# juanaldayparejo/archnemesis-dist

Hardware: AMD Instinct MI355X
Metric: forward-models/sec (10k nu x 100 layers) (higher is better)
Workload: dtype f64; 1 GPU; synthetic correlated-k nadir thermal-emission forward model: 10000 wavenumbers x 100 layers x 8 gases, G=20, k-table 20Px15T (BASELINE configs[1], SURVEY C2); parallelism=replicas x1 (independent forward models)

## Files before the change

archnemesis_dist_amd/csrc/ansfm_api.hip:

```cpp
#include "ansfm_table_kernels.hip.h"
#include "ansfm_rt_params.h"
#include "ansfm_ctx.hip.h"

using namespace ansfm;

extern "C" {

int ansfm_abi_version(void) { return ANSFM_ABI_VERSION; }

int ansfm_create(int device, ansfm_ctx **out)
{
    if (!out) return ANSFM_ERR_INVALID;
    *out = nullptr;
    int ndev = 0;
    if (hipGetDeviceCount(&ndev) != hipSuccess || ndev <= 0 || device < 0 || device >= ndev)
        return ANSFM_ERR_HIP;
    ansfm_ctx *ctx = new ansfm_ctx();
    ctx->device = device;
    if (hipSetDevice(device) != hipSuccess) { delete ctx; return ANSFM_ERR_HIP; }
    if (hipStreamCreateWithFlags(&ctx->own_stream, hipStreamNonBlocking) != hipSuccess) {
        delete ctx;
        return ANSFM_ERR_HIP;
    }
    ctx->stream = ctx->own_stream;
// ... 26 lines not shown
int ansfm_set_gradient_gases(ansfm_ctx *ctx, unsigned int mask)
{
    CHECK_CTX(ctx);
    ctx->grad_gas_mask = mask;
    return ANSFM_OK;
}

int ansfm_set_f32_semantics(ansfm_ctx *ctx, int grid_f32, int delg_f32)
{
    CHECK_CTX(ctx);
    ctx->grid_f32 = grid_f32 ? 1 : 0;
    ctx->delg_f32 = delg_f32 ? 1 : 0;
    return ANSFM_OK;
}

int ansfm_synchronize(ansfm_ctx *ctx)
{
    CHECK_CTX(ctx);
    HIPCHK(hipSetDevice(ctx->device));
    HIPCHK(hipStreamSynchronize(ctx->stream));
    return ANSFM_OK;
}

int ansfm_upload_ktable_dev(ansfm_ctx *ctx, int W, int G, int NP, int NT, int S, const double *K_dev,
                            const double *PRESS, const double *TEMP, const double *WAVE,
                            const double *DELG)
{
    CHECK_CTX(ctx);
    if (W <= 0 || G <= 0 || G > ANSFM_MAX_NG || NP < 2 || NT < 2 || S <= 0 || !K_dev || !PRESS || !TEMP ||
        !WAVE || !DELG)
        FAIL(ANSFM_ERR_INVALID, "upload_ktable: bad dims (need 1<=G<=32, NP>=2, NT>=2) or null pointer");
    HIPCHK(hipSetDevice(ctx->device));
    const int Wpad = round_up(W, kWave);
    const size_t total = (size_t)NP * NT * S * G * Wpad;
    HIPCHK(ctx->lnK.reserve(total * sizeof(double)));
    HIPCHK(ctx->d_press.reserve(NP * sizeof(double)));
    HIPCHK(ctx->d_temp.reserve(NT * sizeof(double)));
    HIPCHK(ctx->d_wave.reserve((size_t)W * sizeof(double)));
    HIPCHK(ctx->d_delg.reserve(kMaxG * sizeof(double)));
    HIPCHK(ctx->d_flag.reserve(kFlagInts * sizeof(int)));
    HIPCHK(hipMemcpyAsync(ctx->d_press.p, PRESS, NP * sizeof(double), hipMemcpyHostToDevice, ctx->stream));
    HIPCHK(hipMemcpyAsync(ctx->d_temp.p, TEMP, NT * sizeof(double), hipMemcpyHostToDevice, ctx->stream));
    HIPCHK(hipMemcpyAsync(ctx->d_wave.p, WAVE, (size_t)W * sizeof(double), hipMemcpyHostToDevice, ctx->stream));
    HIPCHK(hipMemcpyAsync(ctx->d_delg.p, DELG, G * sizeof(double), hipMemcpyHostToDevice, ctx->stream));
    HIPCHK(hipMemsetAsync(ctx->d_flag.p, 0, kFlagInts * sizeof(int), ctx->stream));
    {
        const int Q = NP * NT * S;
        hipLaunchKernelGGL(k_table_check, dim3(nblk((size_t)W * Q, 256)), dim3(256), 0, ctx->stream, K_dev, W, G, Q,
                           ctx->d_flag.as<int>());
        hipLaunchKernelGGL(k_table_relayout, dim3((unsigned)(Wpad / kWave), nblk((size_t)Q, 64), (unsigned)G), dim3(256), 0,
                           ctx->stream, K_dev, ctx->lnK.as<double>(), W, Wpad, G, Q);
    }
    HIPCHK(hipGetLastError());
    int flag = 0;
    HIPCHK(hipMemcpyAsync(&flag, ctx->d_flag.p, sizeof(int), hipMemcpyDeviceToHost, ctx->stream));
    HIPCHK(hipStreamSynchronize(ctx->stream));
    ctx->W = W; ctx->Wpad = Wpad; ctx->G = G; ctx->NP = NP; ctx->NT = NT; ctx->S = S;
    ctx->monotone = (flag & 1) ? 0 : 1;
    ctx->has_boxed = (flag & 2) ? 1 : 0;
    ctx->h_delg.assign(DELG, DELG + G);
    ctx->h_wave.assign(WAVE, WAVE + W); ctx->h_press.assign(PRESS, PRESS + NP); ctx->h_temp.assign(TEMP, TEMP + NT);
    ctx->have_table = true;
    ctx->is_lbl = 0; ctx->temp2d = 0;
    ctx->lblrt = 0; ctx->st_n = 0;
    clear_continuum_sources(ctx);
    return ANSFM_OK;
}

int ansfm_upload_ktable(ansfm_ctx *ctx, int W, int G, int NP, int NT, int S, const double *K,
                        const double *PRESS, const double *TEMP, const double *WAVE, const double *DELG)
{
    CHECK_CTX(ctx);
    if (W <= 0 || G <= 0 || NP <= 0 || NT <= 0 || S <= 0 || !K) FAIL(ANSFM_ERR_INVALID, "upload_ktable: bad dims");
    HIPCHK(hipSetDevice(ctx->device));
    const size_t n = (size_t)W * G * NP * NT * S;
    HIPCHK(ctx->tmp_in.reserve(n * sizeof(double)));
    HIPCHK(hipMemcpyAsync(ctx->tmp_in.p, K, n * sizeof(double), hipMemcpyHostToDevice, ctx->stream));
    int rc = ansfm_upload_ktable_dev(ctx, W, G, NP, NT, S, ctx->tmp_in.as<double>(), PRESS, TEMP, WAVE, DELG);
    ctx->tmp_in.release();
    return rc;
}

namespace {
struct KtaHeader {
    int irec0 = 0, nwave = 0, npress = 0, ntemp = 0, ng = 0, gasID = 0, isoID = 0;
    double vmin = 0, delv = 0, fwhm = 0;
    std::vector<float> g_ord, del_g, press, temp;
    std::vector<double> wave;
    bool temp2d = false;
// ... 119 lines not shown
            FAIL(ANSFM_ERR_INVALID, "upload_ktable_files: " + err);
        if (hs[s].nwave != hs[0].nwave) FAIL(ANSFM_ERR_INVALID, "error :: Number of wavenumbers in all .kta files must be the same");
        if (hs[s].npress != hs[0].npress) FAIL(ANSFM_ERR_INVALID, "error :: Number of pressure levels in all .kta files must be the same");
        if (hs[s].ntemp != hs[0].ntemp) FAIL(ANSFM_ERR_INVALID, "error :: Number of temperature levels in all .kta files must be the same");
        if (hs[s].ng != hs[0].ng) FAIL(ANSFM_ERR_INVALID, "error :: Number of g-ordinates in all .kta files must be the same");
        if (hs[s].temp2d != hs[0].temp2d) FAIL(ANSFM_ERR_INVALID, "error :: Number of temperature levels in all .kta files must be the same");
    }
    const KtaHeader &hl = hs[S - 1];
    const int G = hl.ng, NP = hl.npress, NT = hl.ntemp;
    if (G > ANSFM_MAX_NG || NP < 2 || NT < 2) FAIL(ANSFM_ERR_INVALID, "upload_ktable_files: need 1<=G<=32, NP>=2, NT>=2");
    if (lta && NP > 256) FAIL(ANSFM_ERR_UNSUPPORTED, "upload_lbltable_files: NP <= 256");
    const std::vector<double> &wv = hl.wave;
    long iwl = (long)(std::upper_bound(wv.begin(), wv.end(), wavemin) - wv.begin()) - 1;
    if (iwl < 0) iwl = 0;
    long iwh = (long)(std::lower_bound(wv.begin(), wv.end(), wavemax) - wv.begin());
    if (iwh >= (long)wv.size()) iwh = (long)wv.size() - 1;
    if (iwh < iwl) FAIL(ANSFM_ERR_INVALID, "upload_ktable_files: empty wavenumber range");
    const double wlo = wv[iwl], whi = wv[iwh];
    const int W = (int)(iwh - iwl + 1);
    std::vector<double> WAVE(wv.begin() + iwl, wv.begin() + iwh + 1), PRESS(hl.press.begin(), hl.press.end()),
        TEMP(hl.temp.begin(), hl.temp.end()), DELG(hl.del_g.begin(), hl.del_g.end());
    const int Wpad = round_up(W, kWave);
    const size_t total = (size_t)NP * NT * S * G * Wpad;
    HIPCHK(ctx->lnK.reserve(total * sizeof(double)));
    HIPCHK(ctx->d_press.reserve(NP * sizeof(double)));
    HIPCHK(ctx->d_temp.reserve(TEMP.size() * sizeof(double)));
    HIPCHK(ctx->d_wave.reserve((size_t)W * sizeof(double)));
    HIPCHK(ctx->d_delg.reserve(kMaxG * sizeof(double)));
    HIPCHK(ctx->d_flag.reserve(kFlagInts * sizeof(int)));
    HIPCHK(hipMemcpyAsync(ctx->d_press.p, PRESS.data(), NP * sizeof(double), hipMemcpyHostToDevice, ctx->stream));
    HIPCHK(hipMemcpyAsync(ctx->d_temp.p, TEMP.data(), TEMP.size() * sizeof(double), hipMemcpyHostToDevice, ctx->stream));
    HIPCHK(hipMemcpyAsync(ctx->d_wave.p, WAVE.data(), (size_t)W * sizeof(double), hipMemcpyHostToDevice, ctx->stream));
    HIPCHK(hipMemcpyAsync(ctx->d_delg.p, DELG.data(), G * sizeof(double), hipMemcpyHostToDevice, ctx->stream));
    HIPCHK(hipMemsetAsync(ctx->d_flag.p, 0, kFlagInts * sizeof(int), ctx->stream));
    const size_t per_wave = (size_t)NP * NT * G;
    std::vector<float> block(per_wave * W);
    HIPCHK(ctx->tmp_in.reserve(block.size() * sizeof(float)));
    for (int s = 0; s < S; ++s) {
        const std::vector<double> &ws = hs[s].wave;
        const long a = (long)(std::lower_bound(ws.begin(), ws.end(), wlo) - ws.begin());
        const long b = (long)(std::upper_bound(ws.begin(), ws.end(), whi) - ws.begin());
        if (b - a != W) FAIL(ANSFM_ERR_INVALID, "upload_ktable_files: the tables do not share one wavenumber grid");
        std::string fn(paths[s]);
        const char *ext = lta ? ".lta" : ".kta";
        if (fn.size() < 4 || fn.compare(fn.size() - 4, 4, ext) != 0) fn += ext;
        FILE *f = fopen(fn.c_str(), "rb");
// ... 2 lines not shown
        const bool ok = fseeko(f, (off_t)off, SEEK_SET) == 0 && fread(block.data(), 4, block.size(), f) == block.size();
        fclose(f);
        if (!ok) FAIL(ANSFM_ERR_INVALID, "upload_ktable_files: truncated k data in " + fn);
        HIPCHK(hipMemcpyAsync(ctx->tmp_in.p, block.data(), block.size() * sizeof(float), hipMemcpyHostToDevice, ctx->stream));
        hipLaunchKernelGGL(k_kta_relayout, dim3(nblk(per_wave * Wpad, 256)), dim3(256), 0, ctx->stream, ctx->tmp_in.as<float>(),
                           ctx->lnK.as<double>(), W, Wpad, G, NP, NT, S, s, ctx->d_flag.as<int>());
        HIPCHK(hipGetLastError());
        HIPCHK(hipStreamSynchronize(ctx->stream));
    }
    int flag = 0;
    HIPCHK(hipMemcpyAsync(&flag, ctx->d_flag.p, sizeof(int), hipMemcpyDeviceToHost, ctx->stream));
    HIPCHK(hipStreamSynchronize(ctx->stream));
    ctx->tmp_in.release();
    ctx->W = W; ctx->Wpad = Wpad; ctx->G = G; ctx->NP = NP; ctx->NT = NT; ctx->S = S;
    ctx->monotone = (flag & 1) ? 0 : 1;
    ctx->has_boxed = (flag & 2) ? 1 : 0;
    ctx->h_delg = DELG; ctx->h_wave = WAVE; ctx->h_press = PRESS; ctx->h_temp = TEMP;
    ctx->have_table = true;
    ctx->is_lbl = lta ? 1 : 0; ctx->temp2d = (lta && hl.temp2d) ? 1 : 0;
    ctx->lblrt = 0; ctx->st_n = 0;
    clear_continuum_sources(ctx);
    if (lta) ctx->monotone = 1;
    ctx->grid_f32 = 1; ctx->delg_f32 = lta ? 0 : 1;
    return ANSFM_OK;
}

int ansfm_upload_ktable_files(ansfm_ctx *ctx, int S, const char *const *paths, double wavemin, double wavemax)
{
    return upload_table_files(ctx, S, paths, wavemin, wavemax, false);
}

int ansfm_upload_lbltable_files(ansfm_ctx *ctx, int S, const char *const *paths, double wavemin, double wavemax)
{
    return upload_table_files(ctx, S, paths, wavemin, wavemax, true);
}

int ansfm_ktable_grids(const ansfm_ctx *ctx, double *WAVE, double *PRESS, double *TEMP, double *DELG)
{
    if (!ctx) return ANSFM_ERR_INVALID;
    if (!ctx->have_table) return ANSFM_ERR_NOTABLE;
    if (WAVE) memcpy(WAVE, ctx->h_wave.data(), ctx->h_wave.size() * sizeof(double));
    if (PRESS) memcpy(PRESS, ctx->h_press.data(), ctx->h_press.size() * sizeof(double));
    if (TEMP) memcpy(TEMP, ctx->h_temp.data(), ctx->h_temp.size() * sizeof(double));
    if (DELG) memcpy(DELG, ctx->h_delg.data(), ctx->h_delg.size() * sizeof(double));
    return ANSFM_OK;
}

// ... 6 lines not shown
    return ANSFM_OK;
}

int ansfm_ktable_has_boxed(const ansfm_ctx *ctx, int *has_boxed)
{
    if (!ctx || !has_boxed) return ANSFM_ERR_INVALID;
    if (!ctx->have_table) return ANSFM_ERR_NOTABLE;
    *has_boxed = ctx->has_boxed;
    return ANSFM_OK;
}

int ansfm_last_merge_launch(const ansfm_ctx *ctx, int *waves_per_block, int *trims)
{
    if (!ctx || !waves_per_block || !trims) return ANSFM_ERR_INVALID;
    *waves_per_block = ctx->merge_block_waves;
    *trims = ctx->merge_trims;
    return ANSFM_OK;
}

int ansfm_last_merge_group_width(const ansfm_ctx *ctx, int *width)
{
    if (!ctx || !width) return ANSFM_ERR_INVALID;
    *width = ctx->merge_group_width;
    return ANSFM_OK;
}

int ansfm_last_merge_rowmajor(const ansfm_ctx *cctx, int64_t *merges, int64_t *merges_total)
{
    ansfm_ctx *ctx = const_cast<ansfm_ctx *>(cctx);
    CHECK_CTX(ctx);
    if (!merges || !merges_total) FAIL(ANSFM_ERR_INVALID, "last_merge_rowmajor: null argument");
    *merges = *merges_total = 0;
    if (ctx->d_flag.bytes < kFlagInts * sizeof(int)) return ANSFM_OK;
    HIPCHK(hipSetDevice(ctx->device));
    unsigned long long v[2] = {0, 0};
    HIPCHK(hipMemcpyAsync(v, ctx->d_flag.as<int>() + kFlagTileCounter + 8, sizeof v, hipMemcpyDeviceToHost, ctx->stream));
    HIPCHK(hipStreamSynchronize(ctx->stream));
    *merges = (int64_t)v[0];
    *merges_total = (int64_t)v[1];
    return ANSFM_OK;
}

static void launch_w_to_last(hipStream_t st, unsigned n_batch, const double *src, double *dst, int W, int Wpad, int X1, int X2,
                             int swap12, double padval, size_t src_stride = 0, size_t dst_stride = 0)
{
    const int X = X1 * X2;
// ... 1020 lines not shown
```

archnemesis_dist_amd/csrc/ansfm_ctx.hip.h:

```cpp
#pragma once
#include <hip/hip_runtime.h>
#include <stdio.h>
#include <stdlib.h>
#include <string.h>

#include <algorithm>
#include <cmath>
#include <initializer_list>
#include <memory>
#include <string>
#include <map>
#include <vector>

#pragma GCC visibility push(default)
#include "../../include/ansfm.h"
#pragma GCC visibility pop

namespace ansfm {

struct DevBuf {
    void *p = nullptr;
    size_t bytes = 0;
    DevBuf() = default;
    DevBuf(const DevBuf &) = delete;
// ... 42 lines not shown

struct ansfm_ctx {
    int device = 0;
    hipStream_t own_stream = nullptr;
    hipStream_t stream = nullptr;
    std::string err;
    int num_cus = 256;

    int W = 0, Wpad = 0, G = 0, NP = 0, NT = 0, S = 0;
    int monotone = 0;
    int has_boxed = 1;
    std::vector<double> h_wave, h_press, h_temp;
    DevBuf dcont_gas;
    int dcont_gas_L = 0;
    unsigned grad_gas_mask = 0xFFFFFFFFu;
    std::map<const void *, size_t> merge_lds_allowed;
    int merge_block_waves = 0, merge_trims = 0;
    int merge_group_width = 0;
    int merge_keys = 64;
    bool have_table = false;
    int grid_f32 = 0, delg_f32 = 0;
    int is_lbl = 0, temp2d = 0;
    DevBuf lnK, d_press, d_temp, d_wave, d_delg, d_flag;
    std::vector<double> h_delg;
    DevBuf cia_tab, cia_idx, cia_lay, dust_kext;
    int cia_on = 0, cia_ispace = 0, cia_NWC = 0, cia_NPAIR = 0, cia_NPE = 0, cia_NT = 0, cia_nfrac = 0, cia_NPARA = 0, cia_NVMR = 0,
        cia_ico2 = -1, cia_in2 = -1, cia_ih2 = -1, cia_covers = 0;
    int dust_n = 0;

    DevBuf li, tau, scratch, cont_t, tmp_in, tmp_out, misc;
    DevBuf dspec_ref, map_out, map_b, map_batch;
    DevBuf dd_slot, dd_work, dd_in;
    DevBuf ms_radg16, ms_brdf16;
    DevBuf rt_prefix, rt_same;
    int last_rt_shared = 0;
    int dedup = 1;
    int last_rows = 0, last_dedup = 0;
    int dspec_dims[4] = {0, 0, 0, 0};
    int map_dims[4] = {0, 0, 0, 0};
    DevBuf gscratch, perm, dkbuf, trold_ws, dspec_i, dcont_t, tmp_in2, tmp_out2, lbl_li;
    DevBuf ms_taus, ms_omegas, ms_bnu;
    DevBuf ms_tauray_l, ms_lfrac_l;
    DevBuf ms_cache, ms_orders, ms_same, ms_pcache, ms_lstart;
    long ms_cache_hits = 0, ms_cache_layers = 0;
    long ms_windows = 0, ms_window_w = 0;
    DevBuf hb[24];
// ... 147 lines not shown
```

archnemesis_dist_amd/csrc/ansfm_merge64.hip.h:

```cpp
#pragma once
#include <hip/hip_runtime.h>
#include <stdint.h>
#include "ansfm_merge_common.hip.h"

namespace ansfm {

constexpr unsigned kLdsDG = 0, kLdsGORD = kMaxG * 8, kLdsDGF = (2 * kMaxG + 2) * 8, kLdsA = kLdsDGF + kMaxG * 4;


constexpr int kOptTable = 1, kOptBfi = 2, kOptExit = 8, kOptOrient = 16;
constexpr int kMergeOpt = kOptTable | kOptBfi | kOptExit | kOptOrient;
constexpr int kOptLaneRows = 32;
constexpr int kOptRowMajor = 64;
constexpr int kFlagLaneRows = 1, kFlagRowMajor = 2;
__host__ __device__ constexpr bool merge_opt_valid(int opt) { return opt == 0 || (opt & ~kOptTable) == (kOptBfi | kOptExit | kOptOrient); }
__host__ __device__ constexpr int merge_wave_rows(int G, int opt) { return 2 * G + ((opt & kOptOrient) != 0 ? 2 : 1); }
constexpr unsigned kLdsWT = kLdsA;
constexpr int kMaxBlockWaves = 8;
__host__ __device__ constexpr unsigned weight_table_bytes(int G) { return (unsigned)(G + 1) * 32u * 8u; }
typedef double dbl2 __attribute__((ext_vector_type(2)));
constexpr unsigned kRecRow = 64u * 16u, kRecBin = 2u * kRecRow;

struct MergeElem {
    double ai, bc, bn, w;
    int ci, np;
};

struct MergeOrient {
    unsigned rbase, cbase;
    unsigned rsh, csh;
    unsigned inc;
};
__device__ __forceinline__ MergeOrient merge_orient(unsigned a_addr, unsigned b_addr, bool swapped)
{
    MergeOrient mo;
    mo.rbase = swapped ? b_addr : a_addr; mo.cbase = swapped ? a_addr : b_addr;
    mo.rsh = swapped ? 6u : 0u; mo.csh = swapped ? 0u : 5u; mo.inc = swapped ? 1u : 32u;
// ... 349 lines not shown
```

archnemesis_dist_amd/csrc/ansfm_merge_common.hip.h:

```cpp
#pragma once
#include <hip/hip_runtime.h>
#include <stdint.h>

namespace ansfm {

constexpr int kWave = 64;
constexpr int kMaxG = 32;

__device__ __forceinline__ double encode_lnk(double k)
{
    if (k > 0.0) return log(k);
    unsigned long long b = (unsigned long long)__double_as_longlong(k);
    unsigned long long box = 0x7FF8000000000000ULL | (b >> 13);
    return __longlong_as_double((long long)box);
}
__device__ __forceinline__ bool lnk_is_boxed(double x) { return x != x; }
__device__ __forceinline__ double lnk_unbox(double x)
{
    unsigned long long b = (unsigned long long)__double_as_longlong(x);
    return __longlong_as_double((long long)((b & 0x0007FFFFFFFFFFFFULL) << 13));
}

struct LayerInterp {
    int ipl, iph, itl, ith;
// ... 38 lines not shown
        double dxdt = (-l1 * (1.0 - v) - h1 * v + h2 * v + l2 * (1.0 - v)) * dudt;
        dk = kk * dxdt;
    } else if (b1 & b2 & b3 & b4) {
        double klo1 = lnk_unbox(l1), klo2 = lnk_unbox(l2), khi1 = lnk_unbox(h1), khi2 = lnk_unbox(h2);
        kk = (1.0 - v) * (1.0 - u) * klo1 + v * (1.0 - u) * khi1 + v * u * khi2 + (1.0 - v) * u * klo2;
        dk = (-klo1 * (1.0 - v) - khi1 * v + khi2 * v + klo2 * (1.0 - v)) * dudt;
    }
}


struct OverlapParams {
    const double *lnK;
    const double *kin;
    const LayerInterp *li;
    const double *amount;
    const double *del_g;
    double *tau;
    double *scratch;
    int *err_flag;
    unsigned int *tile_counter;
    int W, Wpad, G, NT, S, L, n_models;
    int delg_f32;
    double g_ord[kMaxG + 2];
};


constexpr int kLoadBatch = 10;

template <bool FROM_K, bool NONNEG = false, bool NOBOX = false>
__device__ __forceinline__ void load_gas(const OverlapParams &p, const LayerInterp &q, int m, int l,
                                         int s, int nu, double *DST, int lane, bool &unsorted)
{
    const int G = p.G;
    const double amt = p.amount[((size_t)m * p.S + s) * p.L + l];
    double prev = NONNEG ? 0.0 : -__builtin_inf();
    if constexpr (FROM_K) {
        const double *src = p.kin + (((size_t)s * p.L + l) * G) * p.Wpad + nu;
        for (int g0 = 0; g0 < G; g0 += kLoadBatch) {
            double r[kLoadBatch];
#pragma unroll
            for (int k = 0; k < kLoadBatch; ++k) {
                const int gi = (g0 + k < G) ? g0 + k : G - 1;
                r[k] = src[(size_t)gi * p.Wpad];
            }
#pragma unroll
            for (int k = 0; k < kLoadBatch; ++k)
                if (g0 + k < G) {
// ... 85 lines not shown
    {0, 0, 100, 2, 0, 0}, {1, 36, 100, 2, 0, 50}, {99, 63, 100, 2, 63, 99}, {50, 17, 100, 2, 33, 8},
    {1, 36, 33, 1, 3, 1}, {32, 63, 33, 1, 63, 32}, {16, 17, 33, 1, 31, 18}, {1, 36, 3, 2, 32, 2}, {2, 63, 3, 2, 63, 2}, {1, 17, 3, 2, 27, 1}};
__host__ __device__ constexpr bool lane_spots_hold()
{
    for (const auto &t : kLaneTileSpots)
        if ((t[2] != 1u && t[2] != (unsigned)kLaneNV) || lane_tile_of(t[0], t[1], t[2] == 1u ? 0u : kLaneNVShift) != t[3]) return false;
    for (const auto &t : kLaneCellSpots) {
        if (t[3] != 1u && t[3] != (unsigned)kLaneNV) return false;
        const LaneCell x = lane_cell(t[0] * 64u + t[1], t[2], t[3] == 1u ? 0u : kLaneNVShift);
        if (x.w != t[4] || x.row != t[5]) return false;
    }
    return true;
}
static_assert(lane_spots_hold(), "lane_tile_of / lane_cell against the model's values");

struct LaneRow {
    int nu;
    unsigned row;
    unsigned arow, krow;
    size_t o1, o2, o3, o4;
    double v, u;
};
template <bool FROM_K>
__device__ __forceinline__ LaneRow lane_row(const OverlapParams &p, int vt, unsigned k, int lane, unsigned nvs)
{
    const unsigned R = (unsigned)p.n_models * (unsigned)p.L;
    const LaneCell cell = lane_cell(k * kWave + (unsigned)lane, R, nvs);
    LaneRow lr;
    lr.row = cell.row;
    lr.nu = vt * kWave + (int)cell.w;
    const unsigned m = lr.row / (unsigned)p.L;
    lr.krow = lr.row - m * (unsigned)p.L;
    lr.arow = m * (unsigned)p.S * (unsigned)p.L + lr.krow;
    lr.o1 = lr.o2 = lr.o3 = lr.o4 = 0;
    lr.v = lr.u = 0.0;
    if constexpr (!FROM_K) {
        const LayerInterp q = p.li[lr.row];
        const size_t strideT = (size_t)p.S * p.G * p.Wpad;
        lr.o1 = ((size_t)q.ipl * p.NT + q.itl) * strideT + lr.nu;
        lr.o2 = ((size_t)q.ipl * p.NT + q.ith) * strideT + lr.nu;
        lr.o3 = ((size_t)q.iph * p.NT + q.itl) * strideT + lr.nu;
        lr.o4 = ((size_t)q.iph * p.NT + q.ith) * strideT + lr.nu;
        lr.v = q.v; lr.u = q.u;
    }
    return lr;
}

template <bool FROM_K, bool NOBOX>
__device__ __forceinline__ void load_gas_rows(const OverlapParams &p, const LaneRow &lr, int s, double *DST, int lane,
                                              bool &unsorted)
{
    const int G = p.G;
    const double amt = p.amount[(size_t)lr.arow + (size_t)s * p.L];
    double prev = -__builtin_inf();
    if constexpr (FROM_K) {
        const double *src = p.kin + (((size_t)s * p.L + lr.krow) * G) * p.Wpad + lr.nu;
        for (int g0 = 0; g0 < G; g0 += kLoadBatch) {
            double r[kLoadBatch];
#pragma unroll
            for (int k = 0; k < kLoadBatch; ++k) {
                const int gi = (g0 + k < G) ? g0 + k : G - 1;
                r[k] = src[(size_t)gi * p.Wpad];
            }
#pragma unroll
            for (int k = 0; k < kLoadBatch; ++k)
                if (g0 + k < G) {
                    const double kk = r[k] * amt;
                    DST[(g0 + k) * kWave + lane] = kk;
                    unsorted |= (kk < prev);
                    prev = kk;
                }
        }
    } else {
        const double *base = p.lnK + (size_t)s * G * p.Wpad;
        const double *c1 = base + lr.o1, *c2 = base + lr.o2, *c3 = base + lr.o3, *c4 = base + lr.o4;
        for (int g0 = 0; g0 < G; g0 += kLoadBatch) {
            double r1[kLoadBatch], r2[kLoadBatch], r3[kLoadBatch], r4[kLoadBatch];
#pragma unroll
            for (int k = 0; k < kLoadBatch; ++k) {
                const int gi = (g0 + k < G) ? g0 + k : G - 1;
                const size_t go = (size_t)gi * p.Wpad;
                r1[k] = c1[go];
                r2[k] = c2[go];
                r3[k] = c3[go];
                r4[k] = c4[go];
            }
#pragma unroll
            for (int k = 0; k < kLoadBatch; ++k)
                if (g0 + k < G) {
                    const double kk = (NOBOX ? interp_k_nobox(r1[k], r2[k], r3[k], r4[k], lr.v, lr.u)
                                             : interp_k(r1[k], r2[k], r3[k], r4[k], lr.v, lr.u)) * amt;
                    DST[(g0 + k) * kWave + lane] = kk;
                    unsorted |= (kk < prev);
                    prev = kk;
                }
        }
    }
}

__device__ __forceinline__ double fast_div(double n, double d)
{
    double r = __builtin_amdgcn_rcp(d);
    r = fma(fma(-d, r, 1.0), r, r);
    r = fma(fma(-d, r, 1.0), r, r);
    double q = n * r;
    return fma(fma(-d, q, n), r, q);
}

// ... 71 lines not shown
```

archnemesis_dist_amd/csrc/ansfm_overlap.hip:

```cpp
#include "ansfm_overlap_kernels.hip.h"
#include "ansfm_merge32_launch.h"
#include "ansfm_ctx.hip.h"

namespace ansfm {

void merge_params(ansfm_ctx *ctx, OverlapParams &p, const double *kin, int W, int Wpad, int G, int S, int L, int n_models,
                  const LayerInterp *li, const double *amount, const double *del_g_dev, const double *del_g_host, double *tau)
{
    p.lnK = ctx->lnK.as<double>();
    p.kin = kin;
    p.li = li;
    p.amount = amount;
    p.del_g = del_g_dev;
    p.tau = tau;
    p.err_flag = ctx->d_flag.as<int>() + 1;
    p.tile_counter = reinterpret_cast<unsigned int *>(ctx->d_flag.as<int>() + kFlagTileCounter);
    p.W = W; p.Wpad = Wpad; p.G = G; p.NT = ctx->NT; p.S = S; p.L = L; p.n_models = n_models;
    p.delg_f32 = ctx->delg_f32;
    double acc = 0.0;
    float accf = 0.0f;
    p.g_ord[0] = 0.0;
    for (int g = 0; g < G; ++g) {
        if (ctx->delg_f32) { accf += (float)del_g_host[g]; p.g_ord[g + 1] = (double)accf; }
        else { acc += del_g_host[g]; p.g_ord[g + 1] = acc; }
// ... 56 lines not shown
    if ((opt & kOptTable) != 0) {
        const size_t shared_bytes = table_bytes + weight_table_bytes(G);
        nwaves = (int)((kCuLdsBytes - shared_bytes) / wave_bytes);
        if (nwaves > max_per_cu) nwaves = max_per_cu;
        if (nwaves > kMaxBlockWaves) nwaves = kMaxBlockWaves;
        lds = shared_bytes + (size_t)nwaves * wave_bytes;
        const int rc = merge_launch_begin(ctx, p, lds, 1, {{&ctx->scratch, (size_t)nwaves * 6 * G * kWave * sizeof(double)}}, &grid);
        if (rc) return rc;
        const long ntiles = (long)n_models * (Wpad / kWave) * L;
        if (grid > (ntiles + nwaves - 1) / nwaves) grid = (ntiles + nwaves - 1) / nwaves;
    } else {
        const int rc = merge_launch_begin(ctx, p, lds_alloc, max_per_cu, {{&ctx->scratch, (size_t)6 * G * kWave * sizeof(double)}}, &grid);
        if (rc) return rc;
    }
    p.scratch = ctx->scratch.as<double>();
    bool lane_rows = opt != 0 && (long)n_models * L < (1L << 24);
    int lane_nv = 1;
    if (const char *ev = getenv("ANSFM_MERGE_LANES")) {
        if (!strcmp(ev, "wavenumbers")) lane_rows = false;
        else if (!strcmp(ev, "pairs")) lane_nv = kLaneNV;
    }
    bool rowmajor = (opt & kOptTable) != 0;
    if (const char *ev = getenv("ANSFM_MERGE_ROWMAJOR")) { if (ev[0] == '0') rowmajor = false; }
    const int flags = (lane_rows ? kFlagLaneRows : 0) | (rowmajor ? kFlagRowMajor : 0);
    ctx->merge_block_waves = nwaves;
    ctx->merge_group_width = lane_rows ? lane_nv : 0;
    ctx->merge_trims = opt == 0 ? 0 : merge_opt_of(ctx->delg_f32 != 0) | (lane_rows ? kOptLaneRows : 0) | (rowmajor ? kOptRowMajor : 0);
    if (keys32) {
        HIPCHK(launch_overlap32(p, from_k, merge_list_len(G), (unsigned)grid, ctx->stream));
        return ANSFM_OK;
    }
#define LAUNCH_OPT(...)                                                                                             \
    do {                                                                                                            \
        auto kern = __VA_ARGS__;                                                                                    \
        size_t &lds_allowed = ctx->merge_lds_allowed[reinterpret_cast<const void *>(kern)];     \
        if (lds > (size_t)64 * 1024 && lds > lds_allowed) {          \
            HIPCHK(hipFuncSetAttribute(reinterpret_cast<const void *>(kern), hipFuncAttributeMaxDynamicSharedMemorySize, (int)lds)); \
            lds_allowed = lds;                                                                                      \
        }                                                                                                           \
        hipLaunchKernelGGL(kern, dim3((unsigned)grid), dim3(kWave * nwaves), lds, ctx->stream, p, flags, lane_nv);           \
    } while (0)
#define LAUNCH_OV2(D, FK, W32)                                                                                      \
    do {                                                                                                            \
        if (opt != 0 && nobox)                                                                                      \
            LAUNCH_OPT(k_ck_overlap<D, false, W32, true, true, true, merge_opt_of(W32)>);                           \
        else if (opt != 0)                                                                                          \
            LAUNCH_OPT(k_ck_overlap<D, FK, W32, true, true, false, merge_opt_of(W32)>);                             \
// ... 32 lines not shown
```

archnemesis_dist_amd/csrc/ansfm_overlap_kernels.hip.h:

```cpp
#pragma once
#include "ansfm_merge64.hip.h"

namespace ansfm {


template <bool FROM_K, bool NOBOX, int OPT>
__device__ __forceinline__ void load_cell(const OverlapParams &p, int lane_rows, const LaneRow &lr, const LayerInterp &q, int m,
                                          int l, int s, int nu, double *DST, int lane, bool &unsorted)
{
    if constexpr (OPT != 0) {
        if (lane_rows != 0) {
            load_gas_rows<FROM_K, NOBOX>(p, lr, s, DST, lane, unsorted);
            return;
        }
    }
    load_gas<FROM_K, false, NOBOX>(p, q, m, l, s, nu, DST, lane, unsorted);
}

template <int NR, bool FROM_K, bool W32, bool SORTED = true, bool NODIV = false, bool NOBOX = false, int OPT = 0>
__global__ __launch_bounds__((OPT & kOptTable) != 0 ? kWave * kMaxBlockWaves : kWave) __attribute__((amdgpu_waves_per_eu(1, 2)))
void k_ck_overlap(OverlapParams p, int flags, int lane_nv)
{
    static_assert(OPT == 0 || (SORTED && NODIV), "the fast path");
    static_assert(merge_opt_valid(OPT), "OPT == 0 || (OPT & ~kOptTable) == (kOptBfi | kOptExit | kOptOrient)");
    constexpr bool kTable = (OPT & kOptTable) != 0, kOrient = (OPT & kOptOrient) != 0;
    static_assert(!kTable || W32, "the weight table holds float32 products only (launch_overlap)");
    const int lane_rows = kTable ? (flags & kFlagLaneRows) : flags;
    const unsigned nvs = lane_nv == 1 ? 0u : kLaneNVShift;
    unsigned n_rowmajor = 0, n_merged = 0;
    extern __shared__ double smem[];
    const int lane = kTable ? (int)(threadIdx.x & 63u) : (int)threadIdx.x;
    const int wv = kTable ? __builtin_amdgcn_readfirstlane((int)(threadIdx.x >> 6)) : 0;
    const int nwv = kTable ? (int)(blockDim.x >> 6) : 1;
    const int G = p.G;
    double *DG = smem;
    double *GORD = DG + kMaxG;
    double *A = reinterpret_cast<double *>(reinterpret_cast<char *>(GORD + kMaxG + 2) + kMaxG * sizeof(float));
    if constexpr (kTable) {
        double *WT = A;
        for (int idx = (int)threadIdx.x; idx < (G + 1) * 32; idx += (int)blockDim.x) {
            const int row = idx & 31, col = idx >> 5;
            double w = 0.0;
            if (row < G && col < G) w = (double)((float)p.del_g[row] * (float)p.del_g[col]);
            WT[idx] = w;
        }
        A = WT + (G + 1) * 32 + (size_t)wv * merge_wave_rows(G, OPT) * kWave;
    }
    double *B = A + (kOrient ? G + 1 : G) * kWave;
    unsigned char *PA = reinterpret_cast<unsigned char *>(B + (G + 1) * kWave);
    unsigned char *PB = PA + G * kWave;
    if (wv == 0 && lane < G) {
        DG[lane] = p.del_g[lane];
        const_cast<float *>(delg_f32_table(DG))[lane] = (float)p.del_g[lane];
    }
    if (wv == 0 && lane < G + 2) GORD[lane] = p.g_ord[lane];
    const double HUGE_KEY = __longlong_as_double(0x7FE0000000000000LL);
    B[G * kWave + lane] = HUGE_KEY;
    if constexpr (kOrient) A[G * kWave + lane] = HUGE_KEY;
    __syncthreads();
    double wsum = 0.0;
    for (int g = 0; g < G; ++g) wsum += DG[g];
    const double wtot = wsum * wsum;

    double *rec = p.scratch + ((size_t)blockIdx.x * nwv + wv) * 6 * G * kWave;
    TileQueue tq;
    tq.init();
    for (;;) {
        int vt = 0, m = 0, l = 0;
        LaneRow lr{};
        if constexpr (OPT != 0) {
            if (lane_rows != 0) {
                unsigned k = 0;
                if (!tq.next_rows(p, lane, nvs, vt, k)) break;
                lr = lane_row<FROM_K>(p, vt, k, lane, nvs);
            } else if (!tq.next(p, lane, vt, m, l)) break;
        } else {
            if (!tq.next(p, lane, vt, m, l)) break;
        }
        const int nu = vt * kWave + lane;
        LayerInterp q;
        if constexpr (!FROM_K) q = p.li[(size_t)m * p.L + l];
        bool unsorted = false;

        load_cell<FROM_K, NOBOX, OPT>(p, lane_rows, lr, q, m, l, 0, nu, A, lane, unsorted);
        double alast = A[(G - 1) * kWave + lane];
        if constexpr (!SORTED) sort_column(A, PA, G, lane);
        for (int s = 1; s < p.S; ++s) {
            load_cell<FROM_K, NOBOX, OPT>(p, lane_rows, lr, q, m, l, s, nu, B, lane, unsorted);
            if constexpr (SORTED)
                if (__builtin_amdgcn_ballot_w64(unsorted) != 0) break;
            const double blast = B[(G - 1) * kWave + lane];
            if constexpr (!SORTED) sort_column(B, PB, G, lane);
            if constexpr (SORTED) alast = A[(G - 1) * kWave + lane];
            bool takeB, keepA;
            if (s == 1) { takeB = (alast <= 0.0); keepA = !takeB && (blast <= 0.0); }
            else { keepA = (blast <= 0.0); takeB = !keepA && (alast <= 0.0); }
            const bool do_merge = !(takeB | keepA);
            bool walked = false;
            if (takeB) {
                for (int g = 0; g < G; ++g) A[g * kWave + lane] = B[g * kWave + lane];
                if constexpr (!SORTED) {
                    for (int g = 0; g < G; ++g) PA[g * kWave + lane] = PB[g * kWave + lane];
                    alast = blast;
                }
            }
            if (do_merge) {
                double R[NR];
                MergeOrient mo{};
                if constexpr (kOrient) {
                    bool swapped = blast > alast;
                    if (__builtin_amdgcn_ballot_w64(swapped) != 0) {
// ... 141 lines not shown
```

archnemesis_dist_amd/csrc/ansfm_table_kernels.hip.h:

```cpp
#pragma once
#include <hip/hip_runtime.h>
#include <stdint.h>
#include "ansfm_merge_common.hip.h"

namespace ansfm {

__global__ void k_layer_prep(int n_layers_total, const double *__restrict__ lay_press_pa,
                             const double *__restrict__ lay_temp, int NP,
                             const double *__restrict__ PRESS, int NT,
                             const double *__restrict__ TEMP, double press_div, int grid_f32,
                             LayerInterp *__restrict__ out)
{
    int i = blockIdx.x * blockDim.x + threadIdx.x;
    if (i >= n_layers_total) return;
    double press1 = lay_press_pa[i] / press_div;
    double temp1 = lay_temp[i];
    int ip = 0;
    double best = fabs(PRESS[0] - press1);
    for (int k = 1; k < NP; ++k) {
        double d = fabs(PRESS[k] - press1);
        if (d < best) { best = d; ip = k; }
    }
    int ipl, iph;
    bool pclamp = false;
// ... 38 lines not shown
    r.ipl = ipl; r.iph = iph; r.itl = itl; r.ith = ith;
    r.v = (lpress - plo) / pden;
    r.u = (temp1 - tlo) / tden;
    if (grid_f32 && pclamp) r.v = (double)(((float)lpress - (float)plo) / (float)pden);
    if (grid_f32 && tclamp) r.u = (double)(((float)temp1 - (float)tlo) / (float)tden);
    r.dudt = dudt;
    out[i] = r;
}

__global__ __launch_bounds__(256) void k_table_relayout(const double *__restrict__ K, double *__restrict__ lnK, int W,
                                                        int Wpad, int G, int Q)
{
    __shared__ double tile[64][65];
    const int tx = threadIdx.x & 63, ty = threadIdx.x >> 6;
    const int w0 = blockIdx.x * 64, q0 = blockIdx.y * 64, g = blockIdx.z;
    for (int r = ty; r < 64; r += 4) {
        const int w = w0 + r, q = q0 + tx;
        tile[r][tx] = (w < W && q < Q) ? K[((size_t)w * G + g) * Q + q] : 0.0;
    }
    __syncthreads();
    for (int r = ty; r < 64; r += 4) {
        const int q = q0 + r;
        if (q < Q) lnK[((size_t)q * G + g) * Wpad + w0 + tx] = encode_lnk(tile[tx][r]);
    }
}

__global__ void k_table_check(const double *__restrict__ K, int W, int G, int Q, int *flag)
{
    const size_t idx = (size_t)blockIdx.x * blockDim.x + threadIdx.x;
    if (idx >= (size_t)W * Q) return;
    const int q = (int)(idx % Q);
    const size_t w = idx / Q;
    const double *src = K + w * (size_t)G * Q + q;
    bool bad = false, boxed = false;
    double prev = 0.0;
    for (int g = 0; g < G; ++g) {
        const double k = src[(size_t)g * Q];
        bad |= !(k >= 0.0) || (g > 0 && k < prev);
        boxed |= !(k > 0.0);
        prev = k;
    }
    if (bad) atomicOr(flag, 1);
    if (boxed) atomicOr(flag, 2);
}

__global__ void k_calc_k_seam(const double *__restrict__ lnK, int W, int Wpad, int G, int NT, int S,
// ... 305 lines not shown
```

archnemesis_dist_amd/engine.py:

```python
import contextlib
import ctypes as C
import os
import numpy as np

from . import _lib

_f8 = np.float64


def _np(a, dtype=_f8):
    return None if a is None else np.ascontiguousarray(a, dtype=dtype)


def _is_f32(a):
    return getattr(a, "dtype", None) == np.float32


def _ptr(a):
    if a is None:
        return None
    if isinstance(a, np.ndarray):
        return a.ctypes.data_as(C.c_void_p)
    return C.c_void_p(a.data_ptr())

# ... 199 lines not shown
                    "calc_klbl_online")
        return k

    def ktable_info(self):
        dims = (C.c_int64 * 5)()
        mono = C.c_int()
        self._check(self._lib.ansfm_ktable_info(self._ctx, dims, C.byref(mono)), "ktable_info")
        return tuple(int(d) for d in dims), bool(mono.value)

    def ktable_has_boxed(self):
        b = C.c_int()
        self._check(self._lib.ansfm_ktable_has_boxed(self._ctx, C.byref(b)), "ktable_has_boxed")
        return bool(b.value)

    def last_merge_launch(self):
        w, t = C.c_int(), C.c_int()
        self._check(self._lib.ansfm_last_merge_launch(self._ctx, C.byref(w), C.byref(t)), "last_merge_launch")
        return int(w.value), int(t.value)

    def last_merge_group_width(self):
        w = C.c_int()
        self._check(self._lib.ansfm_last_merge_group_width(self._ctx, C.byref(w)), "last_merge_group_width")
        return int(w.value)

    def last_merge_rowmajor(self):
        m, t = C.c_int64(), C.c_int64()
        self._check(self._lib.ansfm_last_merge_rowmajor(self._ctx, C.byref(m), C.byref(t)), "last_merge_rowmajor")
        return int(m.value), int(t.value)

    def calc_k(self, press, temp, grad=False):
        press = _np(press); temp = _np(temp)
        W, G, NP, NT, S = self.dims
        L = press.shape[0]
        k = np.empty((W, G, L, S)); dk = np.empty((W, G, L, S)) if grad else None
        self._check(self._lib.ansfm_calc_k(self._ctx, L, _ptr(press), _ptr(temp), _ptr(k), _ptr(dk)), "calc_k")
        return (k, dk) if grad else k

    def k_overlap(self, del_g, k_w_g_l_gas, amount_layer):
        self.set_f32_semantics(getattr(self, "grid_f32", False), _is_f32(del_g))
        del_g = _np(del_g); k = _np(k_w_g_l_gas); am = _np(amount_layer)
        W, G, L, S = k.shape
        if am.shape != (S, L):
            raise ValueError("amount_layer must be (NGAS, NLAYER)")
        tau = np.empty((W, G, L))
        self._check(self._lib.ansfm_k_overlap(self._ctx, W, G, L, S, _ptr(del_g), _ptr(k), _ptr(am), _ptr(tau)),
                    "k_overlap")
# ... 1156 lines not shown
```

include/ansfm.h:

```cpp
#ifndef ANSFM_H
#define ANSFM_H

#include <stdint.h>

#ifdef __cplusplus
extern "C" {
#endif

#define ANSFM_ABI_VERSION 1

#define ANSFM_OK 0
#define ANSFM_ERR_INVALID 1
#define ANSFM_ERR_HIP 2
#define ANSFM_ERR_NOTABLE 3
#define ANSFM_ERR_UNSORTED 4
#define ANSFM_ERR_UNSUPPORTED 5

#define ANSFM_MAX_NG 32

typedef struct ansfm_ctx ansfm_ctx;

int ansfm_abi_version(void);

int ansfm_create(int device, ansfm_ctx **ctx);
void ansfm_destroy(ansfm_ctx *ctx);
const char *ansfm_last_error(const ansfm_ctx *ctx);

int ansfm_set_stream(ansfm_ctx *ctx, void *hip_stream);
int ansfm_synchronize(ansfm_ctx *ctx);

int ansfm_set_f32_semantics(ansfm_ctx *ctx, int grid_f32, int delg_f32);

int ansfm_upload_ktable(ansfm_ctx *ctx, int W, int G, int NP, int NT, int S, const double *K,
                        const double *PRESS, const double *TEMP, const double *WAVE,
                        const double *DELG);
int ansfm_upload_ktable_dev(ansfm_ctx *ctx, int W, int G, int NP, int NT, int S,
                            const double *K_dev, const double *PRESS, const double *TEMP,
                            const double *WAVE, const double *DELG);
int ansfm_ktable_info(const ansfm_ctx *ctx, int64_t dims[5], int *monotone);
int ansfm_ktable_has_boxed(const ansfm_ctx *ctx, int *has_boxed);
int ansfm_last_merge_launch(const ansfm_ctx *ctx, int *waves_per_block, int *trims);
int ansfm_last_merge_rowmajor(const ansfm_ctx *ctx, int64_t *merges, int64_t *merges_total);
int ansfm_last_merge_group_width(const ansfm_ctx *ctx, int *width);

int ansfm_upload_lbltable(ansfm_ctx *ctx, int W, int NP, int NT, int S, const double *K,
                          const double *PRESS, const double *TEMP, int temp2d, const double *WAVE);
int ansfm_calc_klbl(ansfm_ctx *ctx, int L, const double *press, const double *temp, double *k_out,
                    double *dkdT_out);

int ansfm_ktable_file_header(const char *path, int64_t dims[4], int32_t ids[2], double hdr[3], double *wave,
                             float *g_ord, float *del_g, float *press, float *temp);
int ansfm_upload_ktable_files(ansfm_ctx *ctx, int S, const char *const *paths, double wavemin, double wavemax);
int ansfm_ktable_grids(const ansfm_ctx *ctx, double *WAVE, double *PRESS, double *TEMP, double *DELG);
int ansfm_lbltable_file_header(const char *path, int64_t dims[3], int32_t ids[2], double hdr[2], double *wave,
                               float *press, float *temp);
int ansfm_upload_lbltable_files(ansfm_ctx *ctx, int S, const char *const *paths, double wavemin, double wavemax);

int ansfm_kdist_bins(ansfm_ctx *ctx, int ncalc, const double *wavecalc, const double *kabs, int nbin,
                     const double *vbinmin, const double *vbinmax, const double *wcen, int nfilmax,
                     const int32_t *nfil, const double *dfil, const double *afil, int NG, const double *g_ord,
                     double *kout);


int ansfm_calc_k(ansfm_ctx *ctx, int L, const double *press, const double *temp, double *k_out,
                 double *dkdT_out);

// ... 327 lines not shown
```

Baseline: 274.9 forward-models/s.

## Add g-fastest k-table copy and load ordinate pairs in lane-row merge

```diff
diff --git a/archnemesis_dist_amd/csrc/ansfm_api.hip b/archnemesis_dist_amd/csrc/ansfm_api.hip
--- a/archnemesis_dist_amd/csrc/ansfm_api.hip
+++ b/archnemesis_dist_amd/csrc/ansfm_api.hip
@@ -72,6 +72,27 @@
     return ANSFM_OK;
 }
 
+static constexpr bool kTableGfastDefault = true;
+static int build_table_gfast(ansfm_ctx *ctx, int Wpad, int G, int Q, bool lbl)
+{
+    bool want = kTableGfastDefault;
+    if (const char *ev = getenv("ANSFM_TABLE_GFAST")) want = ev[0] == '1' ? true : (ev[0] == '0' ? false : want);
+    ctx->lnKg_bytes = 0;
+    if (!want || lbl || G < 2 || Wpad / kWave > 65535) { ctx->lnKg.release(); return ANSFM_OK; }
+    const size_t bytes = (size_t)Q * Wpad * gfast_stride(G) * sizeof(double);
+    if (ctx->lnKg.reserve(bytes) != hipSuccess) {
+        (void)hipGetLastError();
+        ctx->lnKg.release();
+        return ANSFM_OK;
+    }
+    hipLaunchKernelGGL(k_table_gfast, dim3((unsigned)Q, (unsigned)(Wpad / kWave)), dim3(256), 0, ctx->stream,
+                       ctx->lnK.as<double>(), ctx->lnKg.as<double>(), Wpad, G);
+    HIPCHK(hipGetLastError());
+    HIPCHK(hipStreamSynchronize(ctx->stream));
+    ctx->lnKg_bytes = bytes;
+    return ANSFM_OK;
+}
+
 int ansfm_upload_ktable_dev(ansfm_ctx *ctx, int W, int G, int NP, int NT, int S, const double *K_dev,
                             const double *PRESS, const double *TEMP, const double *WAVE,
                             const double *DELG)
@@ -83,6 +104,7 @@
     HIPCHK(hipSetDevice(ctx->device));
     const int Wpad = round_up(W, kWave);
     const size_t total = (size_t)NP * NT * S * G * Wpad;
+    ctx->lnKg_bytes = 0;
     HIPCHK(ctx->lnK.reserve(total * sizeof(double)));
     HIPCHK(ctx->d_press.reserve(NP * sizeof(double)));
     HIPCHK(ctx->d_temp.reserve(NT * sizeof(double)));
@@ -114,7 +136,7 @@
     ctx->is_lbl = 0; ctx->temp2d = 0;
     ctx->lblrt = 0; ctx->st_n = 0;
     clear_continuum_sources(ctx);
-    return ANSFM_OK;
+    return build_table_gfast(ctx, Wpad, G, NP * NT * S, false);
 }
 
 int ansfm_upload_ktable(ansfm_ctx *ctx, int W, int G, int NP, int NT, int S, const double *K,
@@ -280,6 +302,7 @@
         TEMP(hl.temp.begin(), hl.temp.end()), DELG(hl.del_g.begin(), hl.del_g.end());
     const int Wpad = round_up(W, kWave);
     const size_t total = (size_t)NP * NT * S * G * Wpad;
+    ctx->lnKg_bytes = 0;
     HIPCHK(ctx->lnK.reserve(total * sizeof(double)));
     HIPCHK(ctx->d_press.reserve(NP * sizeof(double)));
     HIPCHK(ctx->d_temp.reserve(TEMP.size() * sizeof(double)));
@@ -328,7 +351,7 @@
     clear_continuum_sources(ctx);
     if (lta) ctx->monotone = 1;
     ctx->grid_f32 = 1; ctx->delg_f32 = lta ? 0 : 1;
-    return ANSFM_OK;
+    return build_table_gfast(ctx, Wpad, G, NP * NT * S, lta);
 }
 
 int ansfm_upload_ktable_files(ansfm_ctx *ctx, int S, const char *const *paths, double wavemin, double wavemax)
@@ -381,6 +404,22 @@
 {
     if (!ctx || !width) return ANSFM_ERR_INVALID;
     *width = ctx->merge_group_width;
+    return ANSFM_OK;
+}
+
+int ansfm_last_merge_table_layout(const ansfm_ctx *ctx, int *gfast)
+{
+    if (!ctx || !gfast) return ANSFM_ERR_INVALID;
+    *gfast = ctx->merge_table_gfast;
+    return ANSFM_OK;
+}
+
+int ansfm_ktable_gfast(const ansfm_ctx *ctx, int *present, int64_t *bytes)
+{
+    if (!ctx || !present || !bytes) return ANSFM_ERR_INVALID;
+    if (!ctx->have_table) return ANSFM_ERR_NOTABLE;
+    *present = ctx->lnKg_bytes != 0 ? 1 : 0;
+    *bytes = (int64_t)ctx->lnKg_bytes;
     return ANSFM_OK;
 }
 
diff --git a/archnemesis_dist_amd/csrc/ansfm_ctx.hip.h b/archnemesis_dist_amd/csrc/ansfm_ctx.hip.h
--- a/archnemesis_dist_amd/csrc/ansfm_ctx.hip.h
+++ b/archnemesis_dist_amd/csrc/ansfm_ctx.hip.h
@@ -88,6 +88,9 @@
     int grid_f32 = 0, delg_f32 = 0;
     int is_lbl = 0, temp2d = 0;
     DevBuf lnK, d_press, d_temp, d_wave, d_delg, d_flag;
+    DevBuf lnKg;
+    size_t lnKg_bytes = 0;
+    int merge_table_gfast = 0;
     std::vector<double> h_delg;
     DevBuf cia_tab, cia_idx, cia_lay, dust_kext;
     int cia_on = 0, cia_ispace = 0, cia_NWC = 0, cia_NPAIR = 0, cia_NPE = 0, cia_NT = 0, cia_nfrac = 0, cia_NPARA = 0, cia_NVMR = 0,
diff --git a/archnemesis_dist_amd/csrc/ansfm_merge64.hip.h b/archnemesis_dist_amd/csrc/ansfm_merge64.hip.h
--- a/archnemesis_dist_amd/csrc/ansfm_merge64.hip.h
+++ b/archnemesis_dist_amd/csrc/ansfm_merge64.hip.h
@@ -13,6 +13,7 @@
 constexpr int kOptLaneRows = 32;
 constexpr int kOptRowMajor = 64;
 constexpr int kFlagLaneRows = 1, kFlagRowMajor = 2;
+constexpr int kFlagTableGfast = 4;
 __host__ __device__ constexpr bool merge_opt_valid(int opt) { return opt == 0 || (opt & ~kOptTable) == (kOptBfi | kOptExit | kOptOrient); }
 __host__ __device__ constexpr int merge_wave_rows(int G, int opt) { return 2 * G + ((opt & kOptOrient) != 0 ? 2 : 1); }
 constexpr unsigned kLdsWT = kLdsA;
diff --git a/archnemesis_dist_amd/csrc/ansfm_merge_common.hip.h b/archnemesis_dist_amd/csrc/ansfm_merge_common.hip.h
--- a/archnemesis_dist_amd/csrc/ansfm_merge_common.hip.h
+++ b/archnemesis_dist_amd/csrc/ansfm_merge_common.hip.h
@@ -84,7 +84,10 @@
     int W, Wpad, G, NT, S, L, n_models;
     int delg_f32;
     double g_ord[kMaxG + 2];
+    const double *lnKg;
 };
+__host__ __device__ constexpr int gfast_stride(int G) { return (G + 1) & ~1; }
+typedef double lnk_pair __attribute__((ext_vector_type(2)));
 
 
 constexpr int kLoadBatch = 10;
@@ -216,7 +219,7 @@
     double v, u;
 };
 template <bool FROM_K>
-__device__ __forceinline__ LaneRow lane_row(const OverlapParams &p, int vt, unsigned k, int lane, unsigned nvs)
+__device__ __forceinline__ LaneRow lane_row(const OverlapParams &p, int vt, unsigned k, int lane, unsigned nvs, bool gfast)
 {
     const unsigned R = (unsigned)p.n_models * (unsigned)p.L;
     const LaneCell cell = lane_cell(k * kWave + (unsigned)lane, R, nvs);
@@ -230,20 +233,22 @@
     lr.v = lr.u = 0.0;
     if constexpr (!FROM_K) {
         const LayerInterp q = p.li[lr.row];
-        const size_t strideT = (size_t)p.S * p.G * p.Wpad;
-        lr.o1 = ((size_t)q.ipl * p.NT + q.itl) * strideT + lr.nu;
-        lr.o2 = ((size_t)q.ipl * p.NT + q.ith) * strideT + lr.nu;
-        lr.o3 = ((size_t)q.iph * p.NT + q.itl) * strideT + lr.nu;
-        lr.o4 = ((size_t)q.iph * p.NT + q.ith) * strideT + lr.nu;
+        const size_t strideT = (size_t)p.S * (gfast ? gfast_stride(p.G) : p.G) * p.Wpad;
+        const size_t own = gfast ? (size_t)lr.nu * gfast_stride(p.G) : (size_t)lr.nu;
+        lr.o1 = ((size_t)q.ipl * p.NT + q.itl) * strideT + own;
+        lr.o2 = ((size_t)q.ipl * p.NT + q.ith) * strideT + own;
+        lr.o3 = ((size_t)q.iph * p.NT + q.itl) * strideT + own;
+        lr.o4 = ((size_t)q.iph * p.NT + q.ith) * strideT + own;
         lr.v = q.v; lr.u = q.u;
     }
     return lr;
 }
 
-template <bool FROM_K, bool NOBOX>
+template <bool FROM_K, bool NOBOX, bool GFAST>
 __device__ __forceinline__ void load_gas_rows(const OverlapParams &p, const LaneRow &lr, int s, double *DST, int lane,
                                               bool &unsorted)
 {
+    constexpr bool gfast = GFAST && !FROM_K;
     const int G = p.G;
     const double amt = p.amount[(size_t)lr.arow + (size_t)s * p.L];
     double prev = -__builtin_inf();
@@ -266,18 +271,35 @@
                 }
         }
     } else {
-        const double *base = p.lnK + (size_t)s * G * p.Wpad;
+        static_assert(kLoadBatch % 2 == 0, "a batch is whole pairs of ordinates");
+        const int Gs = gfast_stride(G);
+        const double *base = gfast ? p.lnKg + (size_t)s * p.Wpad * Gs : p.lnK + (size_t)s * G * p.Wpad;
         const double *c1 = base + lr.o1, *c2 = base + lr.o2, *c3 = base + lr.o3, *c4 = base + lr.o4;
         for (int g0 = 0; g0 < G; g0 += kLoadBatch) {
             double r1[kLoadBatch], r2[kLoadBatch], r3[kLoadBatch], r4[kLoadBatch];
-#pragma unroll
-            for (int k = 0; k < kLoadBatch; ++k) {
-                const int gi = (g0 + k < G) ? g0 + k : G - 1;
-                const size_t go = (size_t)gi * p.Wpad;
-                r1[k] = c1[go];
-                r2[k] = c2[go];
-                r3[k] = c3[go];
-                r4[k] = c4[go];
+            if constexpr (gfast) {
+#pragma unroll
+                for (int k = 0; k < kLoadBatch; k += 2) {
+                    const int gi = (g0 + k < Gs) ? g0 + k : Gs - 2;
+                    const lnk_pair x1 = *reinterpret_cast<const lnk_pair *>(c1 + gi);
+                    const lnk_pair x2 = *reinterpret_cast<const lnk_pair *>(c2 + gi);
+                    const lnk_pair x3 = *reinterpret_cast<const lnk_pair *>(c3 + gi);
+                    const lnk_pair x4 = *reinterpret_cast<const lnk_pair *>(c4 + gi);
+                    r1[k] = x1.x; r1[k + 1] = x1.y;
+                    r2[k] = x2.x; r2[k + 1] = x2.y;
+                    r3[k] = x3.x; r3[k + 1] = x3.y;
+                    r4[k] = x4.x; r4[k + 1] = x4.y;
+                }
+            } else {
+#pragma unroll
+                for (int k = 0; k < kLoadBatch; ++k) {
+                    const int gi = (g0 + k < G) ? g0 + k : G - 1;
+                    const size_t go = (size_t)gi * p.Wpad;
+                    r1[k] = c1[go];
+                    r2[k] = c2[go];
+                    r3[k] = c3[go];
+                    r4[k] = c4[go];
+                }
             }
 #pragma unroll
             for (int k = 0; k < kLoadBatch; ++k)
diff --git a/archnemesis_dist_amd/csrc/ansfm_overlap.hip b/archnemesis_dist_amd/csrc/ansfm_overlap.hip
--- a/archnemesis_dist_amd/csrc/ansfm_overlap.hip
+++ b/archnemesis_dist_amd/csrc/ansfm_overlap.hip
@@ -102,7 +102,12 @@
     }
     bool rowmajor = (opt & kOptTable) != 0;
     if (const char *ev = getenv("ANSFM_MERGE_ROWMAJOR")) { if (ev[0] == '0') rowmajor = false; }
-    const int flags = (lane_rows ? kFlagLaneRows : 0) | (rowmajor ? kFlagRowMajor : 0);
+    bool gfast = lane_rows && !from_k && !keys32 && ctx->lnKg_bytes != 0 && !ctx->is_lbl && W == ctx->W && Wpad == ctx->Wpad &&
+                 G == ctx->G && S == ctx->S;
+    if (const char *ev = getenv("ANSFM_TABLE_LAYOUT")) { if (!strcmp(ev, "wave")) gfast = false; }
+    if (gfast) p.lnKg = ctx->lnKg.as<double>();
+    const int flags = (lane_rows ? kFlagLaneRows : 0) | (rowmajor ? kFlagRowMajor : 0) | (gfast ? kFlagTableGfast : 0);
+    ctx->merge_table_gfast = gfast ? 1 : 0;
     ctx->merge_block_waves = nwaves;
     ctx->merge_group_width = lane_rows ? lane_nv : 0;
     ctx->merge_trims = opt == 0 ? 0 : merge_opt_of(ctx->delg_f32 != 0) | (lane_rows ? kOptLaneRows : 0) | (rowmajor ? kOptRowMajor : 0);
diff --git a/archnemesis_dist_amd/csrc/ansfm_overlap_kernels.hip.h b/archnemesis_dist_amd/csrc/ansfm_overlap_kernels.hip.h
--- a/archnemesis_dist_amd/csrc/ansfm_overlap_kernels.hip.h
+++ b/archnemesis_dist_amd/csrc/ansfm_overlap_kernels.hip.h
@@ -5,12 +5,13 @@
 
 
 template <bool FROM_K, bool NOBOX, int OPT>
-__device__ __forceinline__ void load_cell(const OverlapParams &p, int lane_rows, const LaneRow &lr, const LayerInterp &q, int m,
+__device__ __forceinline__ void load_cell(const OverlapParams &p, int lane_rows, bool gfast, const LaneRow &lr, const LayerInterp &q, int m,
                                           int l, int s, int nu, double *DST, int lane, bool &unsorted)
 {
     if constexpr (OPT != 0) {
         if (lane_rows != 0) {
-            load_gas_rows<FROM_K, NOBOX>(p, lr, s, DST, lane, unsorted);
+            if (!FROM_K && gfast) load_gas_rows<FROM_K, NOBOX, true>(p, lr, s, DST, lane, unsorted);
+            else load_gas_rows<FROM_K, NOBOX, false>(p, lr, s, DST, lane, unsorted);
             return;
         }
     }
@@ -26,6 +27,7 @@
     constexpr bool kTable = (OPT & kOptTable) != 0, kOrient = (OPT & kOptOrient) != 0;
     static_assert(!kTable || W32, "the weight table holds float32 products only (launch_overlap)");
     const int lane_rows = kTable ? (flags & kFlagLaneRows) : flags;
+    const bool gfast = !FROM_K && OPT != 0 && (flags & kFlagTableGfast) != 0;
     const unsigned nvs = lane_nv == 1 ? 0u : kLaneNVShift;
     unsigned n_rowmajor = 0, n_merged = 0;
     extern __shared__ double smem[];
@@ -72,7 +74,7 @@
             if (lane_rows != 0) {
                 unsigned k = 0;
                 if (!tq.next_rows(p, lane, nvs, vt, k)) break;
-                lr = lane_row<FROM_K>(p, vt, k, lane, nvs);
+                lr = lane_row<FROM_K>(p, vt, k, lane, nvs, gfast);
             } else if (!tq.next(p, lane, vt, m, l)) break;
         } else {
             if (!tq.next(p, lane, vt, m, l)) break;
@@ -82,11 +84,11 @@
         if constexpr (!FROM_K) q = p.li[(size_t)m * p.L + l];
         bool unsorted = false;
 
-        load_cell<FROM_K, NOBOX, OPT>(p, lane_rows, lr, q, m, l, 0, nu, A, lane, unsorted);
+        load_cell<FROM_K, NOBOX, OPT>(p, lane_rows, gfast, lr, q, m, l, 0, nu, A, lane, unsorted);
         double alast = A[(G - 1) * kWave + lane];
         if constexpr (!SORTED) sort_column(A, PA, G, lane);
         for (int s = 1; s < p.S; ++s) {
-            load_cell<FROM_K, NOBOX, OPT>(p, lane_rows, lr, q, m, l, s, nu, B, lane, unsorted);
+            load_cell<FROM_K, NOBOX, OPT>(p, lane_rows, gfast, lr, q, m, l, s, nu, B, lane, unsorted);
             if constexpr (SORTED)
                 if (__builtin_amdgcn_ballot_w64(unsorted) != 0) break;
             const double blast = B[(G - 1) * kWave + lane];
diff --git a/archnemesis_dist_amd/csrc/ansfm_table_kernels.hip.h b/archnemesis_dist_amd/csrc/ansfm_table_kernels.hip.h
--- a/archnemesis_dist_amd/csrc/ansfm_table_kernels.hip.h
+++ b/archnemesis_dist_amd/csrc/ansfm_table_kernels.hip.h
@@ -84,6 +84,23 @@
     for (int r = ty; r < 64; r += 4) {
         const int q = q0 + r;
         if (q < Q) lnK[((size_t)q * G + g) * Wpad + w0 + tx] = encode_lnk(tile[tx][r]);
+    }
+}
+
+__global__ __launch_bounds__(256) void k_table_gfast(const double *__restrict__ lnK, double *__restrict__ lnKg, int Wpad, int G)
+{
+    __shared__ double tile[kMaxG][65];
+    const int Gs = gfast_stride(G);
+    const int tx = threadIdx.x & 63, ty = threadIdx.x >> 6;
+    const size_t q = blockIdx.x;
+    const int w0 = blockIdx.y * 64;
+    for (int g = ty; g < G; g += 4) tile[g][tx] = lnK[(q * G + g) * Wpad + w0 + tx];
+    __syncthreads();
+    const double boxed0 = __longlong_as_double(0x7FF8000000000000LL);
+    double *dst = lnKg + (q * Wpad + w0) * Gs;
+    for (int i = threadIdx.x; i < 64 * Gs; i += 256) {
+        const int w = i / Gs, g = i - w * Gs;
+        dst[i] = g < G ? tile[g][w] : boxed0;
     }
 }
 
diff --git a/archnemesis_dist_amd/engine.py b/archnemesis_dist_amd/engine.py
--- a/archnemesis_dist_amd/engine.py
+++ b/archnemesis_dist_amd/engine.py
@@ -245,6 +245,16 @@
         w = C.c_int()
         self._check(self._lib.ansfm_last_merge_group_width(self._ctx, C.byref(w)), "last_merge_group_width")
         return int(w.value)
+
+    def ktable_gfast(self):
+        p, b = C.c_int(), C.c_int64()
+        self._check(self._lib.ansfm_ktable_gfast(self._ctx, C.byref(p), C.byref(b)), "ktable_gfast")
+        return bool(p.value), int(b.value)
+
+    def last_merge_table_layout(self):
+        g = C.c_int()
+        self._check(self._lib.ansfm_last_merge_table_layout(self._ctx, C.byref(g)), "last_merge_table_layout")
+        return bool(g.value)
 
     def last_merge_rowmajor(self):
         m, t = C.c_int64(), C.c_int64()
diff --git a/include/ansfm.h b/include/ansfm.h
--- a/include/ansfm.h
+++ b/include/ansfm.h
@@ -42,6 +42,8 @@
 int ansfm_last_merge_launch(const ansfm_ctx *ctx, int *waves_per_block, int *trims);
 int ansfm_last_merge_rowmajor(const ansfm_ctx *ctx, int64_t *merges, int64_t *merges_total);
 int ansfm_last_merge_group_width(const ansfm_ctx *ctx, int *width);
+int ansfm_ktable_gfast(const ansfm_ctx *ctx, int *present, int64_t *bytes);
+int ansfm_last_merge_table_layout(const ansfm_ctx *ctx, int *gfast);
 
 int ansfm_upload_lbltable(ansfm_ctx *ctx, int W, int NP, int NT, int S, const double *K,
                           const double *PRESS, const double *TEMP, int temp2d, const double *WAVE);
```

Measured after the change: 280.9 forward-models/s (median of 6 runs). 1.02x the previous value.
